# krisbrud/gym-auv

Hardware: AMD Instinct MI355X
Metric: env-steps/sec (higher is better)
Workload: dtype f64; 1 GPU; 4096 envs x 180 sensors per GPU, 50 static polygon obstacles (BASELINE configs[2]); envs_per_gpu=4096, n_sensors=180, total_envs=4096, parallelism=env-shard x1 (no step-path collective), ranks=1, hipgraph_steps=0, steps_per_launch=64, sub_batches=1, api=multi, step_mode=one_launch, roofline_step_mode=one_launch, actions=uniform, worlds_per_env=2, collective_backend=none, episodes_finished=212

## Files before the change

gym_auv_amd/csrc/k_step_fused.hip:

```cpp
#include <cstdlib>
#include <hip/hip_ext.h>

#define AUV_DEVICE_FUNCS_ONLY
#include "auv_multi_geom.h"
#include "k1_dynamics.hip"
#include "k2_lidar.hip"
#include "k3_nav_reward.hip"

#ifndef AUV_K23_MIN_WAVES
#define AUV_K23_MIN_WAVES 4
#endif

#ifdef AUV_TEST_HOOKS
#define AUV_HOOK_SKEW(d) ((d).pair_skew)
#define AUV_HOOK_FAULT(d) ((d).pair_fault)
#else
#define AUV_HOOK_SKEW(d) 0
#define AUV_HOOK_FAULT(d) 0
#endif

namespace {

#define PAIR_EMPTY AUV_PAIR_EMPTY
#define PAIR_COLLISION AUV_PAIR_COLLISION
// ... 13 lines not shown
  }
}

__device__ __forceinline__ void pair_publish_lidar(const AuvDev& d, const int e, const int lane, const int collision,
                                                   const double term) {
  auv_stores_done();
  if (AUV_HOOK_FAULT(d) == 1 && e == d.e0) return;
  if (lane == 0)
    __hip_atomic_store(d.pair_word + e, collision ? PAIR_COLLISION : (unsigned long long)__double_as_longlong(term),
                       __ATOMIC_RELAXED, __HIP_MEMORY_SCOPE_AGENT);
}

__global__ void __launch_bounds__(AUV_BLOCK, AUV_K23_MIN_WAVES) k23_lidar_nav(AuvDev dk, float* __restrict__ obs_out) {
  const AuvDev& d = dk;
  extern __shared__ __align__(16) unsigned char smem[];
  const int lane = threadIdx.x;
  const int ne = d.ne;
  if ((int)blockIdx.x >= ne) {
    const int el = (int)blockIdx.x - ne;
    if (el >= ne) return;
    const int e = auv_uniform(d.e0 + el);
#ifdef AUV_STAMPS
    const unsigned long long t_nav0 = wall_clock64();
#endif
    k3_nav_env(d, e, lane, smem, obs_out);
#ifdef AUV_STAMPS
    if (lane == 0) d.stamps[(size_t)e * 16 + 12] = t_nav0, d.stamps[(size_t)e * 16 + 13] = wall_clock64();
#endif
  } else {
    const int e = auv_uniform(d.e0 + (int)blockIdx.x);
    if (e == d.e0 && lane == 0 && dk.ring_slots > 1 && dk.ring_slot_host == -1) *dk.ring_pos = (*dk.ring_pos + 1) % dk.ring_slots;
    const Slice L = carve(smem, d);
    AUV_STAMP_DECL
#ifdef AUV_STAMPS
    const unsigned long long t_real0 = wall_clock64();
#endif
    int2 lim0 = make_int2(INT32_MIN, INT32_MIN);
    const int n_act = k2_front(d, e, lane, L, 1, nullptr, 0, nullptr, false, d.cfg.use_lidar ? &lim0 : nullptr);
    if (d.cfg.use_lidar) {
      AUV_STAMP()
#ifdef AUV_STAMPS
      unsigned long long sub[4] = {0, 0, 0, 0};
      k2_stage_and_pairs(d, L, lane, n_act, d.state[2 * (size_t)d.n + e], sub);
      if (lane == 0) d.stamps[(size_t)e * 16 + 7] = sub[0], d.stamps[(size_t)e * 16 + 14] = sub[1], d.stamps[(size_t)e * 16 + 15] = sub[2], d.stamps[(size_t)e * 16 + 6] = sub[3];
#else
      k2_stage_and_pairs(d, L, lane, n_act, d.state[2 * (size_t)d.n + e]);
#endif
      AUV_STAMP()
      double term = 0.0;
      k2_back(d, e, lane, L, n_act, obs_out, &term, &lim0);
      AUV_STAMP()
      AUV_STAMP_FLUSH(e, 0)
#ifdef AUV_STAMPS
      if (lane == 0) d.stamps[(size_t)e * 16 + 3] = t_real0, d.stamps[(size_t)e * 16 + 4] = wall_clock64();
      if (lane == 0) d.stamps[(size_t)e * 16 + 5] = (unsigned long long)L.sbase[n_act];
#endif
    }
  }
}

__device__ __forceinline__ double pair_lane_value(const unsigned long long v, const int src) {
  const unsigned lo = (unsigned)__builtin_amdgcn_readlane((int)(unsigned)v, src);
  const unsigned hi = (unsigned)__builtin_amdgcn_readlane((int)(unsigned)(v >> 32), src);
  return __longlong_as_double((long long)(((unsigned long long)hi << 32) | lo));
}

#define ROLES_MAGIC 0x9e3779b97f4a7c15ull
__device__ __forceinline__ unsigned long long roles_mark(const unsigned long long x) { return (x ^ ROLES_MAGIC) | 1ull; }

__device__ __forceinline__ unsigned long long roles_group_xor(const unsigned long long w) {
  int lo = (int)(unsigned)w, hi = (int)(unsigned)(w >> 32);
  lo ^= __builtin_amdgcn_update_dpp(0, lo, 0xB1, 0xF, 0xF, true), hi ^= __builtin_amdgcn_update_dpp(0, hi, 0xB1, 0xF, 0xF, true);
  lo ^= __builtin_amdgcn_update_dpp(0, lo, 0x4E, 0xF, 0xF, true), hi ^= __builtin_amdgcn_update_dpp(0, hi, 0x4E, 0xF, 0xF, true);
  lo ^= __builtin_amdgcn_update_dpp(0, lo, 0x141, 0xF, 0xF, true), hi ^= __builtin_amdgcn_update_dpp(0, hi, 0x141, 0xF, 0xF, true);
  return ((unsigned long long)(unsigned)hi << 32) | (unsigned)lo;
}

__device__ __forceinline__ unsigned long long roles_lane_word(const unsigned long long v, const int src) {
  return ((unsigned long long)(unsigned)__builtin_amdgcn_readlane((int)(unsigned)(v >> 32), src) << 32) |
         (unsigned)__builtin_amdgcn_readlane((int)(unsigned)v, src);
}

__device__ __forceinline__ unsigned long long roles_tagmix(const unsigned long long tag) { return tag * 0xd6e8feb86659fd93ull; }
__device__ __forceinline__ int roles_wait_state(const AuvDev& d, const int e, const int lane, EnvPre& pre, const unsigned long long tagmix = 0ull,
                                                const bool have_first = false, const unsigned long long v_first = 0ull) {
  const unsigned long long* pk = d.k1_pkt + 8 * (size_t)e;
  unsigned long long v = 0;
  for (int polls = 0;; polls++) {
    if (have_first && polls == 0) v = v_first;
    else v = __hip_atomic_load(pk + (lane & 7), __ATOMIC_RELAXED, __HIP_MEMORY_SCOPE_AGENT);
    const unsigned long long got = roles_lane_word(v, 7);
    if (got != 0ull) {
      unsigned long long x = roles_lane_word(v, 0);
#pragma unroll
      for (int i = 1; i < 7; i++) x ^= roles_lane_word(v, i);
      if (roles_mark(x ^ tagmix) == got) break;
    }
    if (polls == (AUV_HOOK_FAULT(d) ? (1 << 12) : PAIR_POLL_LIMIT)) {
      if (lane == 0) auv_st<true>(d.broken + e, (uint8_t)1);
      roles_give_up(d, d.e0, d.ne, 2, lane);
      return 1;
    }
    __builtin_amdgcn_s_sleep(ROLES_POLL_SLEEP);
  }
#pragma unroll
  for (int i = 0; i < 6; i++) pre.s[i] = pair_lane_value(v, i);
  pre.cnt.y = (int)__builtin_amdgcn_readlane((int)(unsigned)v, 6);
  return (unsigned)pre.cnt.y == ROLES_ABORT_COUNTER ? 2 : 0;
}

__device__ __forceinline__ void roles_publish_search(const AuvDev& d, const int e, const int lane, const NavNear& nr, const unsigned long long tagmix = 0ull) {
  unsigned long long* h = d.nav_hand + 8 * (size_t)e;
  const unsigned long long w0 = (unsigned long long)__double_as_longlong(nr.A.x), w1 = (unsigned long long)__double_as_longlong(nr.A.y),
                           w2 = (unsigned long long)__double_as_longlong(nr.B.x), w3 = (unsigned long long)__double_as_longlong(nr.B.y),
                           w4 = (unsigned long long)__double_as_longlong(nr.cum);
  if (AUV_HOOK_FAULT(d) == 3 && e == d.e0) return;
  if (lane == 0) {
    __hip_atomic_store(h + 0, w0, __ATOMIC_RELAXED, __HIP_MEMORY_SCOPE_AGENT), __hip_atomic_store(h + 1, w1, __ATOMIC_RELAXED, __HIP_MEMORY_SCOPE_AGENT);
    __hip_atomic_store(h + 2, w2, __ATOMIC_RELAXED, __HIP_MEMORY_SCOPE_AGENT), __hip_atomic_store(h + 3, w3, __ATOMIC_RELAXED, __HIP_MEMORY_SCOPE_AGENT);
    __hip_atomic_store(h + 4, w4, __ATOMIC_RELAXED, __HIP_MEMORY_SCOPE_AGENT);
    __hip_atomic_store(h + 7, roles_mark(w0 ^ w1 ^ w2 ^ w3 ^ w4 ^ tagmix), __ATOMIC_RELAXED, __HIP_MEMORY_SCOPE_AGENT);
  }
}

__device__ __forceinline__ unsigned long long roles_group_word(const unsigned long long v, const int src) {
  const unsigned lo = (unsigned)__shfl((int)(unsigned)v, src, K1_GROUP), hi = (unsigned)__shfl((int)(unsigned)(v >> 32), src, K1_GROUP);
  return ((unsigned long long)hi << 32) | lo;
}
__device__ __forceinline__ double roles_group_value(const unsigned long long v, const int src) {
  return __longlong_as_double((long long)roles_group_word(v, src));
}
__device__ __forceinline__ bool roles_record_ok(const unsigned long long v, const int c, const unsigned long long tagmix = 0ull) {
  const unsigned long long x = roles_group_xor(c < 7 ? v : 0ull), mark = roles_group_word(v, 7);
  return mark != 0ull && roles_mark(x ^ tagmix) == mark;
}

__device__ __forceinline__ void roles_finish_wave(const AuvDev& dk, const int f, const int lane, float* __restrict__ obs_out,
                                                  float* __restrict__ reward_out, uint8_t* __restrict__ done_out) {
  const __attribute__((address_space(4))) AuvDev* dc = (const __attribute__((address_space(4))) AuvDev*)dk.self;
  const AuvDev& d = *(const AuvDev*)dc;
  StepTabs st;
  st.cfg.min_cumulative_reward = dc->cfg.min_cumulative_reward, st.cfg.min_goal_distance = dc->cfg.min_goal_distance;
  st.cfg.min_path_progress = dc->cfg.min_path_progress, st.cfg.look_ahead_distance = dc->cfg.look_ahead_distance;
  st.cfg.max_timesteps = dc->cfg.max_timesteps, st.cfg.rewarder = dc->cfg.rewarder, st.cfg.test_mode = dc->cfg.test_mode;
  st.cfg.auto_reset = dc->cfg.auto_reset, st.cfg.n_sensors = dc->cfg.n_sensors, st.cfg.use_lidar = dc->cfg.use_lidar;
  st.cfg.obs_channels = dc->cfg.obs_channels, st.pool_ns = dc->pool_ns;
  st.knot_s = dc->knot_s, st.knot_coef = dc->knot_coef;
  st.info64 = dc->info64, st.nav64 = dc->nav64, st.obs64 = dc->obs64, st.rew_path = dc->rew_path, st.reward64 = dc->reward64;
  st.step_info = dc->step_info, st.episode = dc->episode, st.ep_log = dc->ep_log, st.ep_log_count = dc->ep_log_count;
  st.ep_log_cap = dc->ep_log_cap, st.world_idx = dc->world_idx, st.counters = dc->counters;
  st.fw_serial = dc->fw_serial, st.n = dc->n;
  st.ring_slots = 1, st.ring_slot_host = 0, st.ring_pos = nullptr;
  unsigned long long* const pair_word = dc->pair_word;
  unsigned long long* const k1_pkt = dc->k1_pkt;
  unsigned long long* const nav_hand = dc->nav_hand;
  const EnvDesc* const env_desc = dc->env_desc;
  const double* const world_scalar = dc->world_scalar;
  double* const state = dc->state;
  const int n_envs = dc->n;
  const int ne = dk.ne, e0 = dk.e0;
  const int g = lane / K1_GROUP, c = lane % K1_GROUP;
  const int er = 8 * (8 * (f / 8) + g) + (f % 8);
  const bool live = er < ne;
  const int e = e0 + (live ? er : ne - 1);
  int4 cnt = st.counters[e];
  const int w = st.world_idx[e];
  const double cum_in = st.info64[8 * (size_t)e + 4], cte_sum_in = st.info64[8 * (size_t)e + 7];
  const EnvDesc ed = env_desc[e];
  TailIn t;
  t.kn0 = ed.kn0, t.nk = ed.nk;
  {
    const double* ws = world_scalar + 8 * (size_t)ed.w;
    t.L = ws[0], t.goal_x = ws[1], t.goal_y = ws[2];
    t.knot_first = st.knot_s[ed.kn0], t.knot_last = st.knot_s[ed.kn0 + ed.nk - 1];
    t.maxp_in = st.info64[8 * (size_t)e + 5];
  }
  const unsigned long long* pk = k1_pkt + 8 * (size_t)e;
  unsigned long long* hd = nav_hand + 8 * (size_t)e;
  const int limit = AUV_HOOK_FAULT(dk) ? (1 << 12) : PAIR_POLL_LIMIT;
#ifdef AUV_STAMPS
// ... 128 lines not shown
    if (b - nk >= ne) return;
    const int e = auv_uniform(d.e0 + b - nk);
#ifdef AUV_STAMPS
    if (lane == 0) d.stamps[(size_t)e * 16 + 3] = wall_clock64();
#endif
    if (auv_uniform(*d.abort_flag)) return;
    ed = d.env_desc[e];
    pre.cnt = d.counters[e];
    pre.ed = &ed;
    const Slice L = carve(smem, d);
    k2_movers<true>(d, e, lane, L, ed, 1);
    const K2Pre kp = k2_prefetch(d, e, lane, ed);
    k2_stage_beams(d, lane, L);
#ifdef AUV_STAMPS
    if (lane == 0) d.stamps[(size_t)e * 16 + 1] = wall_clock64();
#endif
    {
      const int ws = roles_wait_state(d, e, lane, pre);
      if (ws) {
        if (ws == 2 && ed.M > 0 && lane == 0) auv_st<true>(d.broken + e, (uint8_t)1);
        return;
      }
    }
#ifdef AUV_STAMPS
    if (lane == 0) d.stamps[(size_t)e * 16 + 2] = wall_clock64();
#endif
    int n_act = 0;
    int2 lim0 = make_int2(INT32_MIN, INT32_MIN);
    if (AUV_RUN_L(d, 1)) n_act = k2_front<true>(d, e, lane, L, 1, &pre, 1, &kp, true, &lim0);
#ifdef AUV_STAMPS
    if (lane == 0) d.stamps[(size_t)e * 16 + 8] = wall_clock64();
#endif
    if (AUV_RUN_L(d, 3)) k2_stage_and_pairs(d, L, lane, n_act, pre.s[2]);
#ifdef AUV_STAMPS
    if (lane == 0) d.stamps[(size_t)e * 16 + 11] = wall_clock64();
#endif
    double term = 0.0;
    const int collision = k2_back<true>(d, e, lane, L, n_act, obs_out, &term, &lim0);
#ifdef AUV_STAMPS
    if (lane == 0) d.stamps[(size_t)e * 16 + 4] = wall_clock64();
#endif
    pair_publish_lidar(d, e, lane, collision, term);
#ifdef AUV_STAMPS
    if (lane == 0) d.stamps[(size_t)e * 16 + 14] = wall_clock64();
#endif
  } else if (b < nk + 2 * nb + AUV_HOOK_SKEW(d)) {
    const int el = b - nk - nb - AUV_HOOK_SKEW(d);
    if (el < 0 || el >= ne) return;
    const int e = auv_uniform(d.e0 + el);
    ed = d.env_desc[e];
    pre.cnt = d.counters[e];
    pre.ed = &ed;
#ifdef AUV_STAMPS
    if (lane == 0) d.stamps[(size_t)e * 16 + 12] = wall_clock64();
#endif
    if (roles_wait_state(d, e, lane, pre)) return;
#ifdef AUV_STAMPS
    if (lane == 0) d.stamps[(size_t)e * 16 + 5] = wall_clock64();
#endif
    NavNear nr;
    nr.A = nr.B = make_double2(0.0, 0.0), nr.cum = 0.0;
    if (AUV_RUN_N(d, 1)) {
      int* list = (int*)smem;
      const NavSpec sp = nav_bounds(d, e, lane, list, pre.s[0], pre.s[1], &ed);
      if (AUV_RUN_N(d, 2)) nr = nav_nearest(d, e, lane, list, pre.s[0], pre.s[1], sp);
    }
    roles_publish_search(d, e, lane, nr);
#ifdef AUV_STAMPS
    if (lane == 0) d.stamps[(size_t)e * 16 + 6] = wall_clock64();
#endif
  } else {
    const int f = b - nk - 2 * nb - AUV_HOOK_SKEW(d);
    if (f < 0 || f >= nk) return;
    __builtin_amdgcn_s_setprio(2);
    roles_finish_wave(d, f, lane, obs_out, reward_out, done_out);
  }
}

#define CARRY_WORDS 24

#ifdef AUV_STAMPS_MULTI
#define MSTAMP(e, k) do { if (lane == 0) stamp[(size_t)(e) * 16 + (k)] = wall_clock64(); } while (0)
#define MSTAMP_IF(cond, e, k) do { if (cond) stamp[(size_t)(e) * 16 + (k)] = wall_clock64(); } while (0)
#define MSTAMP_PARAM , unsigned long long* stamp
#define MSTAMP_ARG , stamp
#else
#define MSTAMP(e, k) do { } while (0)
#define MSTAMP_IF(cond, e, k) do { } while (0)
#define MSTAMP_PARAM
#define MSTAMP_ARG
#endif

__device__ __forceinline__ unsigned long long carry_ed_word(const EnvDesc& ed, const int i) {
  switch (i) {
    case 0: return (unsigned long long)ed.k0;
    case 1: return (unsigned long long)ed.m0;
    case 2: return (unsigned long long)ed.p0;
    case 3: return (unsigned long long)ed.c0;
    case 4: return (unsigned long long)ed.kn0;
    case 5: return (unsigned long long)(unsigned)ed.K | ((unsigned long long)(unsigned)ed.M << 32);
    case 6: return (unsigned long long)(unsigned)ed.P | ((unsigned long long)(unsigned)ed.nch << 32);
    default: return (unsigned long long)(unsigned)ed.nk | ((unsigned long long)(unsigned)ed.w << 32);
  }
}
__device__ __forceinline__ void carry_ed_from(EnvDesc& ed, const unsigned long long w[8]) {
  ed.k0 = (long long)w[0], ed.m0 = (long long)w[1], ed.p0 = (long long)w[2], ed.c0 = (long long)w[3], ed.kn0 = (long long)w[4];
  ed.K = (int)(unsigned)w[5], ed.M = (int)(unsigned)(w[5] >> 32), ed.P = (int)(unsigned)w[6], ed.nch = (int)(unsigned)(w[6] >> 32);
  ed.nk = (int)(unsigned)w[7], ed.w = (int)(unsigned)(w[7] >> 32);
}

__device__ __forceinline__ int carry_wait_wave(const AuvDev& d, const int e, const int lane, const unsigned long long tagmix, EnvDesc& ed, int4& cnt) {
  const unsigned long long* cw = d.carry + CARRY_WORDS * (size_t)e;
  unsigned long long v = 0ull;
  for (int polls = 0;; polls++) {
    if (lane < CARRY_WORDS) v = __hip_atomic_load(cw + lane, __ATOMIC_RELAXED, __HIP_MEMORY_SCOPE_AGENT);
    const unsigned long long ma = roles_lane_word(v, 7), mb = roles_lane_word(v, 20);
    if (ma != 0ull && mb != 0ull) {
      unsigned long long xa = roles_lane_word(v, 0), xb = roles_lane_word(v, 8);
#pragma unroll
      for (int i = 1; i < 7; i++) xa ^= roles_lane_word(v, i);
#pragma unroll
      for (int i = 9; i < 20; i++) xb ^= roles_lane_word(v, i);
      if (roles_mark(xa ^ tagmix) == ma && roles_mark(xb ^ tagmix) == mb) break;
    }
    if ((polls & 31) == 31 && auv_uniform(__hip_atomic_load(d.abort_flag, __ATOMIC_RELAXED, __HIP_MEMORY_SCOPE_AGENT))) return 2;
    if (polls == (AUV_HOOK_FAULT(d) ? (1 << 12) : PAIR_POLL_LIMIT)) {
      if (lane == 0) auv_st<true>(d.broken + e, (uint8_t)1);
      roles_give_up(d, d.e0, d.ne, 6, lane);
      return 1;
    }
    __builtin_amdgcn_s_sleep(ROLES_POLL_SLEEP);
  }
  unsigned long long w[8];
#pragma unroll
  for (int i = 0; i < 8; i++) w[i] = roles_lane_word(v, 12 + i);
  carry_ed_from(ed, w);
  const unsigned long long c6 = roles_lane_word(v, 6), c8 = roles_lane_word(v, 8);
  cnt = make_int4((int)(unsigned)c6, (int)(unsigned)(c6 >> 32), (int)(unsigned)c8, 0);
  return 0;
}

template <bool MULTI>
__device__ __forceinline__ void roles_finish_wave_multi(const AuvDev& dk, const int f, const int lane, float* __restrict__ obs_out,
                                                        float* __restrict__ reward_out, uint8_t* __restrict__ done_out, const int step,
                                                        const bool last_step, const unsigned long long tagmix, const unsigned long long tagmix_prev MSTAMP_PARAM) {
  const __attribute__((address_space(4))) AuvDev* dc = (const __attribute__((address_space(4))) AuvDev*)dk.self;
  const AuvDev& d = *(const AuvDev*)dc;
  StepTabs st;
  st.cfg.min_cumulative_reward = dc->cfg.min_cumulative_reward, st.cfg.min_goal_distance = dc->cfg.min_goal_distance;
  st.cfg.min_path_progress = dc->cfg.min_path_progress, st.cfg.look_ahead_distance = dc->cfg.look_ahead_distance;
  st.cfg.max_timesteps = dc->cfg.max_timesteps, st.cfg.rewarder = dc->cfg.rewarder, st.cfg.test_mode = dc->cfg.test_mode;
  st.cfg.auto_reset = dc->cfg.auto_reset, st.cfg.n_sensors = dc->cfg.n_sensors, st.cfg.use_lidar = dc->cfg.use_lidar;
  st.cfg.obs_channels = dc->cfg.obs_channels, st.pool_ns = dc->pool_ns;
  st.knot_s = dc->knot_s, st.knot_coef = dc->knot_coef;
  st.info64 = dc->info64, st.nav64 = dc->nav64, st.obs64 = dc->obs64, st.rew_path = dc->rew_path, st.reward64 = dc->reward64;
  st.step_info = dc->step_info, st.episode = dc->episode, st.ep_log = dc->ep_log, st.ep_log_count = dc->ep_log_count;
  st.ep_log_cap = dc->ep_log_cap, st.world_idx = dc->world_idx, st.counters = dc->counters;
  st.fw_serial = nullptr, st.n = dc->n;
  st.ring_slots = 1, st.ring_slot_host = 0, st.ring_pos = nullptr;
  unsigned long long* const pair_word = dc->pair_word;
  unsigned long long* const k1_pkt = dc->k1_pkt;
  unsigned long long* const nav_hand = dc->nav_hand;
  unsigned long long* const carry = dc->carry;
  const EnvDesc* const env_desc = dc->env_desc;
  const double* const world_scalar = dc->world_scalar;
  double* const state = dc->state;
  uint8_t* const broken = dc->broken;
  const int n_envs = dc->n;
  const int ne = dk.ne, e0 = dk.e0;
  const int g = lane / K1_GROUP, c = lane % K1_GROUP;
  const int er = 8 * (8 * (f / 8) + g) + (f % 8);
  const bool live = er < ne;
  const int e = e0 + (live ? er : ne - 1);
  const int limit = AUV_HOOK_FAULT(dk) ? (1 << 12) : PAIR_POLL_LIMIT;
  int4 cnt;
  double cum_in, cte_sum_in, maxp_in;
  EnvDesc ed;
  unsigned long long* const cw = carry + CARRY_WORDS * (size_t)e;
  if (step == 0) {
    cnt = st.counters[e];
    cum_in = st.info64[8 * (size_t)e + 4], cte_sum_in = st.info64[8 * (size_t)e + 7], maxp_in = st.info64[8 * (size_t)e + 5];
    ed = env_desc[e];
  } else {
    unsigned long long v0 = 0ull, v1 = 0ull, v2 = 0ull;
    bool ok = !live;
    for (int polls = 0;; polls++) {
      if (!ok) {
        v0 = __hip_atomic_load(cw + c, __ATOMIC_RELAXED, __HIP_MEMORY_SCOPE_AGENT);
        v1 = __hip_atomic_load(cw + 8 + c, __ATOMIC_RELAXED, __HIP_MEMORY_SCOPE_AGENT);
        v2 = __hip_atomic_load(cw + 16 + c, __ATOMIC_RELAXED, __HIP_MEMORY_SCOPE_AGENT);
      }
      const unsigned long long xb = roles_group_xor(v1) ^ roles_group_xor(c < 4 ? v2 : 0ull), mb = roles_group_word(v2, 4);
      ok = !live || (roles_record_ok(v0, c, tagmix_prev) && mb != 0ull && roles_mark(xb ^ tagmix_prev) == mb);
      if (!__any(!ok)) break;
      if ((polls & 31) == 31 && auv_uniform(__hip_atomic_load(dc->abort_flag, __ATOMIC_RELAXED, __HIP_MEMORY_SCOPE_AGENT))) return;
      if (polls == limit) {
        if (live && c == 0) auv_st<true>(broken + e, (uint8_t)1);
        roles_give_up(d, e0, ne, 6, lane);
        return;
      }
      __builtin_amdgcn_s_sleep(ROLES_POLL_SLEEP);
    }
    const unsigned long long c6 = roles_group_word(v0, 6), c8 = roles_group_word(v1, 0);
    cnt = make_int4((int)(unsigned)c6, (int)(unsigned)(c6 >> 32), (int)(unsigned)c8, 0);
    cum_in = roles_group_value(v1, 1), maxp_in = roles_group_value(v1, 2), cte_sum_in = roles_group_value(v1, 3);
    unsigned long long w[8];
#pragma unroll
    for (int i = 0; i < 4; i++) w[i] = roles_group_word(v1, 4 + i);
#pragma unroll
    for (int i = 0; i < 4; i++) w[4 + i] = roles_group_word(v2, i);
    carry_ed_from(ed, w);
    if (!live) ed = env_desc[e];
  }
  const int w = ed.w;
  TailIn t;
  t.kn0 = ed.kn0, t.nk = ed.nk;
  {
    const double* ws = world_scalar + 8 * (size_t)ed.w;
    t.L = ws[0], t.goal_x = ws[1], t.goal_y = ws[2];
    t.knot_first = st.knot_s[ed.kn0], t.knot_last = st.knot_s[ed.kn0 + ed.nk - 1];
    t.maxp_in = maxp_in;
  }
  const unsigned long long* pk = k1_pkt + 8 * (size_t)e;
  unsigned long long* hd = nav_hand + 8 * (size_t)e;
  unsigned long long vp = 0ull, vh = 0ull;
  bool okp = !live, okh = !live, aborted = false;
  for (int polls = 0;; polls++) {
    if (!okp) vp = __hip_atomic_load(pk + c, __ATOMIC_RELAXED, __HIP_MEMORY_SCOPE_AGENT);
    if (!okh) vh = __hip_atomic_load(hd + c, __ATOMIC_RELAXED, __HIP_MEMORY_SCOPE_AGENT);
    okp = !live || roles_record_ok(vp, c, tagmix);
    aborted = live && okp && (unsigned)roles_group_word(vp, 6) == ROLES_ABORT_COUNTER;
    okh = !live || aborted || roles_record_ok(vh, c, tagmix);
    if (!__any(!(okp && okh))) break;
    if (polls == limit) {
      if (live && c == 0) auv_st<true>(broken + e, (uint8_t)1);
      roles_give_up(d, e0, ne, 3, lane);
      return;
    }
    __builtin_amdgcn_s_sleep(ROLES_POLL_SLEEP);
  }
  if (__any(aborted)) return;
  t.px = roles_group_value(vp, 0), t.py = roles_group_value(vp, 1), t.psi = roles_group_value(vp, 2);
  t.u = roles_group_value(vp, 3), t.v = roles_group_value(vp, 4), t.r = roles_group_value(vp, 5);
  cnt.y = (int)(unsigned)roles_group_word(vp, 6);
  t.nr.A = make_double2(roles_group_value(vh, 0), roles_group_value(vh, 1));
  t.nr.B = make_double2(roles_group_value(vh, 2), roles_group_value(vh, 3));
  t.nr.cum = roles_group_value(vh, 4);
  NavOut no;
  no.rew_path = no.reached = no.goal = no.progress = no.u = no.v = no.r = no.cte100 = no.maxp = 0.0;
  unsigned long long word = live ? __hip_atomic_load(pair_word + e, __ATOMIC_RELAXED, __HIP_MEMORY_SCOPE_AGENT) : 0ull;
  no = nav_tail<K1_GROUP>(st, e, c, live, t, obs_out);
  if (live && c < 6) state[(size_t)c * (size_t)n_envs + e] = __longlong_as_double((long long)vp);
  for (int polls = 0;; polls++) {
    if (!__any(word == PAIR_EMPTY)) break;
    if (word == PAIR_EMPTY) word = __hip_atomic_load(pair_word + e, __ATOMIC_RELAXED, __HIP_MEMORY_SCOPE_AGENT);
    if (!__any(word == PAIR_EMPTY)) break;
    if (polls == limit) {
      if (live && c == 0) auv_st<true>(broken + e, (uint8_t)1);
      roles_give_up(d, e0, ne, 1, lane);
      return;
    }
    __builtin_amdgcn_s_sleep(ROLES_POLL_SLEEP);
  }
  MSTAMP_IF(live && c == 0, e, 14);
  int do_reset = 0;
  double co[2] = {0.0, 0.0};
  if (live && c == 0) {
    __hip_atomic_store(pair_word + e, PAIR_EMPTY, __ATOMIC_RELAXED, __HIP_MEMORY_SCOPE_AGENT);
    __hip_atomic_store(k1_pkt + 8 * (size_t)e + 7, 0ull, __ATOMIC_RELAXED, __HIP_MEMORY_SCOPE_AGENT);
    __hip_atomic_store(hd + 7, 0ull, __ATOMIC_RELAXED, __HIP_MEMORY_SCOPE_AGENT);
    RewardIn in;
    const int collision = word == PAIR_COLLISION;
    in.closeness_reward = collision ? 0.0 : __longlong_as_double((long long)word);
    in.path_reward = no.rew_path, in.reached = no.reached, in.goal = no.goal, in.progress = no.progress;
    in.u = no.u, in.v = no.v, in.yaw_rate = no.r;
    in.cum = cum_in;
    in.cte100 = no.cte100, in.cte_sum = cte_sum_in;
    st.info64[8 * (size_t)e] = collision;
    do_reset = reward_apply(st, e, collision, cnt, in, reward_out, done_out, false, co);
  }
  unsigned long long m = __ballot(do_reset);
  const unsigned long long m_reset = m;
  while (m) {
    const int src = __ffsll((long long)m) - 1;
    m &= m - 1;
    const int er2 = auv_uniform(__shfl(e, src, AUV_WAVE));
    const int wr = auv_uniform(__shfl(w, src, AUV_WAVE)), ep = auv_uniform(__shfl(cnt.z, src, AUV_WAVE));
    const AuvDev* dp = dk.self;
    asm volatile("" : "+s"(dp));
    const AuvDev& dr = *(const AuvDev*)(const __attribute__((address_space(4))) AuvDev*)dp;
    restore_env<false, true>(dr, er2, (int)(((long long)wr + dr.n) % dr.n_worlds), lane, ep, obs_out);
  }
  if (last_step) return;
  auv_stores_done();
  unsigned long long w0, w1, w2;
  {
    const int cx = __shfl(cnt.x, 0, K1_GROUP), cy = __shfl(cnt.y, 0, K1_GROUP), cz = __shfl(cnt.z, 0, K1_GROUP);
    const double cum = __shfl(co[0], 0, K1_GROUP), cte = __shfl(co[1], 0, K1_GROUP), maxp = __shfl(no.maxp, 0, K1_GROUP);
    w0 = c < 6 ? vp : (unsigned long long)(unsigned)cx | ((unsigned long long)(unsigned)cy << 32);
    w1 = c == 0 ? (unsigned long long)(unsigned)cz
                : (c == 1 ? (unsigned long long)__double_as_longlong(cum)
                          : (c == 2 ? (unsigned long long)__double_as_longlong(maxp) : (c == 3 ? (unsigned long long)__double_as_longlong(cte) : carry_ed_word(ed, c - 4))));
    w2 = c < 4 ? carry_ed_word(ed, 4 + c) : 0ull;
  }
  if (m_reset & (0xffull << (8 * g))) {
    const size_t n = (size_t)n_envs;
    const int4 rc = make_int4(0, 0, __shfl(cnt.z, 0, K1_GROUP), 0);
    const EnvDesc ne_ = auv_make_desc<true>(d, (int)(((long long)w + d.n) % d.n_worlds));
    const double sv = c < 6 ? __hip_atomic_load(state + (size_t)c * n + e, __ATOMIC_RELAXED, __HIP_MEMORY_SCOPE_AGENT) : 0.0;
    const double iv = (c >= 1 && c <= 3) ? __hip_atomic_load(st.info64 + 8 * (size_t)e + (c == 1 ? 4 : (c == 2 ? 5 : 7)), __ATOMIC_RELAXED, __HIP_MEMORY_SCOPE_AGENT) : 0.0;
    w0 = c < 6 ? (unsigned long long)__double_as_longlong(sv) : 0ull;
    w1 = c == 0 ? (unsigned long long)(unsigned)rc.z : (c <= 3 ? (unsigned long long)__double_as_longlong(iv) : carry_ed_word(ne_, c - 4));
    w2 = c < 4 ? carry_ed_word(ne_, 4 + c) : 0ull;
  }
  const unsigned long long ma = roles_mark(roles_group_xor(c < 7 ? w0 : 0ull) ^ tagmix);
  const unsigned long long mb = roles_mark(roles_group_xor(w1) ^ roles_group_xor(c < 4 ? w2 : 0ull) ^ tagmix);
  if (live) {
    __hip_atomic_store(cw + c, c < 7 ? w0 : ma, __ATOMIC_RELAXED, __HIP_MEMORY_SCOPE_AGENT);
    __hip_atomic_store(cw + 8 + c, w1, __ATOMIC_RELAXED, __HIP_MEMORY_SCOPE_AGENT);
    __hip_atomic_store(cw + 16 + c, c < 4 ? w2 : (c == 4 ? mb : 0ull), __ATOMIC_RELAXED, __HIP_MEMORY_SCOPE_AGENT);
  }
}

#define AUV_KERNARG_DESC(name)                                                                                                                       \
  const __attribute__((address_space(4))) void* name##_kp_ = (const __attribute__((address_space(4))) void*)__builtin_amdgcn_kernarg_segment_ptr(); \
  asm volatile("" : "+s"(name##_kp_));                                                                                                               \
  const AuvDev& name = *(const AuvDev*)(const __attribute__((address_space(4))) AuvDev*)name##_kp_

__global__ void __launch_bounds__(AUV_WAVE, AUV_K23_MIN_WAVES) k_step_multi(AuvDev dk, const void* __restrict__ actions, float* __restrict__ obs_out,
                                                                           float* __restrict__ reward_out, uint8_t* __restrict__ done_out,
                                                                           const int n_steps, const int first_slot, const int n_slots,
                                                                           const unsigned long long seq0, const int lead_dyn, const int lag_fin, const unsigned magic_c) {
  AUV_KERNARG_DESC(d);
#define STEP_MULTI_REC 0
#include "k_step_multi_body.inc"
#undef STEP_MULTI_REC
}

__global__ void __launch_bounds__(AUV_WAVE, AUV_K23_MIN_WAVES) k_step_record(AuvDev dk, const void* __restrict__ actions, float* __restrict__ obs_out,
                                                                            float* __restrict__ reward_out, uint8_t* __restrict__ done_out,
                                                                            const int n_steps, const int first_slot, const int n_slots,
                                                                            const unsigned long long seq0, const int lead_dyn, const int lag_fin, const unsigned magic_c,
                                                                            const unsigned long long obs_stride, const unsigned long long reward_stride,
                                                                            const unsigned long long done_stride) {
  AUV_KERNARG_DESC(d);
#define STEP_MULTI_REC 1
#include "k_step_multi_body.inc"
#undef STEP_MULTI_REC
}

__global__ void __launch_bounds__(256) k_record_last(const float* __restrict__ obs_last, const float* __restrict__ reward_last,
                                                     const uint8_t* __restrict__ done_last, float* __restrict__ obs, float* __restrict__ reward,
                                                     uint8_t* __restrict__ done, const int e0, const int ne, const int D, const int32_t* __restrict__ abort_flag) {
  if (*abort_flag) return;
  const size_t i = (size_t)blockIdx.x * 256 + threadIdx.x;
  const size_t o0 = (size_t)e0 * (size_t)D;
  if (obs_last && i < (size_t)ne * (size_t)D) obs[o0 + i] = obs_last[o0 + i];
  if (i < (size_t)ne) reward[e0 + i] = reward_last[e0 + i], done[e0 + i] = done_last[e0 + i];
}

__global__ void __launch_bounds__(AUV_WAVE) k31_reward_dyn(AuvDev d, const void* __restrict__ actions, float* __restrict__ obs_out,
                                                           float* __restrict__ reward_out, uint8_t* __restrict__ done_out) {
  const int lane = threadIdx.x;
  const int e = blockIdx.x * AUV_WAVE + lane;
  int do_reset = 0, w = 0;
  int4 cnt = make_int4(0, 0, 0, 0);
  if (e < d.n) {
    cnt = d.counters[e];
    w = d.world_idx[e];
    const int collision = d.collision[e];
    d.info64[8 * (size_t)e] = collision;
    do_reset = reward_block(d, e, collision, cnt, false, 0.0, nullptr, reward_out, done_out, false);
  }
  unsigned long long m = __ballot(do_reset);
  const bool any_reset = m != 0;
  while (m) {
    const int src = __ffsll((long long)m) - 1;
    m &= m - 1;
    const int er = auv_uniform(__shfl(e, src, AUV_WAVE));
    const int wr = auv_uniform(__shfl(w, src, AUV_WAVE)), ep = __shfl(cnt.z, src, AUV_WAVE);
    restore_env(d, er, auv_next_world_wave(d, wr, lane), lane, ep, obs_out);
  }
  if (any_reset) __builtin_amdgcn_fence(__ATOMIC_ACQ_REL, "workgroup");
  if (e < d.n) k1_env(d, e, actions, true);
}

__global__ void __launch_bounds__(AUV_WAVE) k_probe_order(unsigned int* __restrict__ words, int np, int nc, unsigned int tag,
                                                          unsigned int* __restrict__ failures) {
  extern __shared__ __align__(16) unsigned char smem[];
  const int b = (int)blockIdx.x, lane = threadIdx.x;
  if (lane == 0) smem[0] = 1;
  unsigned int* mine = words + b;
  const unsigned int* src = nullptr;
  if (b >= np + 2 * nc) {
    const int q = b - np - 2 * nc;
    if (lane < 8) src = words + np + nc + 8 * q + lane;
    else if (lane < 16) src = words + np + 8 * q + (lane - 8);
    else if (lane < 24) src = words + (8 * q + (lane - 16)) % np;
  } else if (b >= np + nc) src = words + np + (b - np - nc);
  else if (b >= np) src = words + (b - np) % np;
  if (b >= np) {
    int polls = 0;
    for (;;) {
      const bool there = !src || __hip_atomic_load(src, __ATOMIC_RELAXED, __HIP_MEMORY_SCOPE_AGENT) == tag;
// ... 146 lines not shown
```

gym_auv_amd/csrc/k_step_multi_body.inc:

```
  extern __shared__ __align__(16) unsigned char smem[];
#ifdef AUV_STAMPS_MULTI
  const unsigned long long t_entry = wall_clock64();
#endif
  const int lane = threadIdx.x;
  const int ne = d.ne;
  const bool cohorts = lead_dyn >= 0;
  const AuvMultiWave wa = auv_multi_decode_steps(blockIdx.x, ne, n_steps);
  const AuvMultiWave wc = auv_multi_decode_cohorts(blockIdx.x, ne, n_steps, lead_dyn, lag_fin, magic_c);
  const int step = auv_uniform(cohorts ? wc.step : wa.step);
  const int role = auv_uniform(cohorts ? wc.role : wa.role), bi = auv_uniform(cohorts ? wc.bi : wa.bi);
  if (step >= n_steps) return;
#if STEP_MULTI_REC
  {
    obs_out += (unsigned long long)(unsigned)step * obs_stride;
    reward_out += (unsigned long long)(unsigned)step * reward_stride;
    done_out += (unsigned long long)(unsigned)step * done_stride;
  }
#endif
  const unsigned long long tagmix = roles_tagmix(seq0 + (unsigned long long)step + 1ull), tagmix_prev = roles_tagmix(seq0 + (unsigned long long)step);
#ifdef AUV_STAMPS_MULTI
  unsigned long long* const stamp = d.stamps + (step == n_steps / 2 ? (size_t)0 : (size_t)16 * (size_t)d.n);
#endif
  if (role == 0) {
    __builtin_amdgcn_s_setprio(3);
    const int b = bi;
    const int g = lane / K1_GROUP, c = lane % K1_GROUP;
    const int er = 8 * (8 * (b / 8) + g) + (b % 8);
    const bool live = er < ne;
    const int eg = d.e0 + (live ? er : ne - 1);
    int y, gave_up = 0;
    double y0 = 0.0;
    MSTAMP_IF(live && c == 0, eg, 10);
    const int ab_early = __hip_atomic_load(d.abort_flag, __ATOMIC_RELAXED, __HIP_MEMORY_SCOPE_AGENT);
    double act0, act1;
    k1_action(d, actions, eg, &act0, &act1, (first_slot + step) % n_slots);
    if (step == 0) {
      y = d.counters[eg].y + 1;
    } else {
      const unsigned long long* cw = d.carry + CARRY_WORDS * (size_t)eg;
      unsigned long long v = 0ull;
      bool ok = !live;
      for (int polls = 0;; polls++) {
        if (!ok) v = __hip_atomic_load(cw + c, __ATOMIC_RELAXED, __HIP_MEMORY_SCOPE_AGENT);
        ok = !live || roles_record_ok(v, c, tagmix_prev);
        if (!__any(!ok)) break;
        if ((polls & 31) == 31 && auv_uniform(__hip_atomic_load(d.abort_flag, __ATOMIC_RELAXED, __HIP_MEMORY_SCOPE_AGENT))) {
          gave_up = 1;
          break;
        }
        if (polls == (AUV_HOOK_FAULT(d) ? (1 << 12) : PAIR_POLL_LIMIT)) {
          if (live && c == 0) auv_st<true>(d.broken + eg, (uint8_t)1);
          roles_give_up(d, d.e0, d.ne, 6, lane);
          gave_up = 1;
          break;
        }
        __builtin_amdgcn_s_sleep(ROLES_POLL_SLEEP);
      }
      y0 = __longlong_as_double((long long)v);
      y = (int)(unsigned)(roles_group_word(v, 6) >> 32) + 1;
    }
    const int aborted = gave_up | auv_uniform(ab_early);
    double t = 0.0;
    MSTAMP_IF(live && c == 0, eg, 11);
    const double2 act = make_double2(act0, act1);
    if (!aborted) t = k1_group(d, actions, eg, lane, step == 0 ? nullptr : &y0, (first_slot + step) % n_slots, &act);
    unsigned long long* pk = d.k1_pkt + 8 * (size_t)eg;
    const unsigned long long word = aborted ? (c == 6 ? (unsigned long long)ROLES_ABORT_COUNTER : 0ull)
                                            : (c < 6 ? (unsigned long long)__double_as_longlong(t) : (c == 6 ? (unsigned long long)(unsigned)y : 0ull));
    const unsigned long long mark = roles_mark(roles_group_xor(word) ^ tagmix);
    if (live && !(AUV_HOOK_FAULT(d) == 2 && eg == d.e0 && step == 0))
      __hip_atomic_store(pk + c, c < 7 ? word : mark, __ATOMIC_RELAXED, __HIP_MEMORY_SCOPE_AGENT);
    MSTAMP_IF(live && c == 0, eg, 12);
    return;
  }
  EnvPre pre;
  EnvDesc ed;
  if (role == 1) {
    const int e = auv_uniform(d.e0 + bi);
    MSTAMP(e, 0);
    const int ab_early = __hip_atomic_load(d.abort_flag, __ATOMIC_RELAXED, __HIP_MEMORY_SCOPE_AGENT);
    const unsigned long long pk_first = __hip_atomic_load(d.k1_pkt + 8 * (size_t)e + (lane & 7), __ATOMIC_RELAXED, __HIP_MEMORY_SCOPE_AGENT);
    const Slice L = carve(smem, d);
    K2Pre kp;
    if (step == 0) {
      ed = d.env_desc[e];
      pre.cnt = d.counters[e];
      pre.ed = &ed;
      if (auv_uniform(ab_early)) return;
      k2_movers<true>(d, e, lane, L, ed, 1);
      kp = k2_prefetch(d, e, lane, ed);
    } else {
      if (carry_wait_wave(d, e, lane, tagmix_prev, ed, pre.cnt)) return;
      if (auv_uniform(ab_early)) return;
      pre.ed = &ed;
      k2_movers<true, true>(d, e, lane, L, ed, 1);
      kp = k2_prefetch<true>(d, e, lane, ed);
    }
    k2_stage_beams(d, lane, L);
    {
      const int ws = roles_wait_state(d, e, lane, pre, tagmix, true, pk_first);
      if (ws) {
        if (ws == 2 && ed.M > 0 && lane == 0) auv_st<true>(d.broken + e, (uint8_t)1);
        return;
      }
    }
    MSTAMP(e, 2);
    int2 lim0 = make_int2(INT32_MIN, INT32_MIN);
    const int n_act = k2_front<true>(d, e, lane, L, 1, &pre, 1, &kp, true, &lim0);
    k2_stage_and_pairs(d, L, lane, n_act, pre.s[2]);
    MSTAMP(e, 4);
    double term = 0.0;
    const int collision = k2_back<true>(d, e, lane, L, n_act, obs_out, &term, &lim0);
    pair_publish_lidar(d, e, lane, collision, term);
    MSTAMP(e, 5);
#ifdef AUV_STAMPS_MULTI
    if (lane == 0) stamp[(size_t)e * 16 + 1] = t_entry;
    __builtin_amdgcn_s_waitcnt(0x0F70);
    MSTAMP(e, 3);
#endif
  } else if (role == 2) {
    const int e = auv_uniform(d.e0 + bi);
    MSTAMP(e, 6);
    const unsigned long long pk_first = __hip_atomic_load(d.k1_pkt + 8 * (size_t)e + (lane & 7), __ATOMIC_RELAXED, __HIP_MEMORY_SCOPE_AGENT);
    if (step == 0) {
      ed = d.env_desc[e];
      pre.cnt = d.counters[e];
    } else if (carry_wait_wave(d, e, lane, tagmix_prev, ed, pre.cnt)) {
      return;
    }
#ifdef AUV_STAMPS_MULTI
    if (lane == 0) stamp[(size_t)e * 16 + 7] = t_entry;
#endif
    pre.ed = &ed;
    if (roles_wait_state(d, e, lane, pre, tagmix, true, pk_first)) return;
    MSTAMP(e, 8);
    NavNear nr;
    int* list = (int*)smem;
    const NavSpec sp = nav_bounds(d, e, lane, list, pre.s[0], pre.s[1], &ed);
    nr = nav_nearest(d, e, lane, list, pre.s[0], pre.s[1], sp);
    roles_publish_search(d, e, lane, nr, tagmix);
    MSTAMP(e, 9);
  } else {
    const int f = bi;
    __builtin_amdgcn_s_setprio(2);
#ifdef AUV_STAMPS_MULTI
    const int fer = 8 * (8 * (f / 8) + lane / K1_GROUP) + (f % 8);
    const bool fst = fer < ne && lane % K1_GROUP == 0;
#endif
    MSTAMP_IF(fst, d.e0 + fer, 13);
    roles_finish_wave_multi<true>(d, f, lane, obs_out, reward_out, done_out, step, step == n_steps - 1, tagmix, tagmix_prev MSTAMP_ARG);
    MSTAMP_IF(fst, d.e0 + fer, 15);
  }
```

Measured before the change: 185.1 million env-steps/s.

## Fuse next-step dynamics into finish wave, drop dedicated dynamics waves after step 0

The finish wave now computes the next step's action and dynamics (k1_group) right after writing the carry, and publishes the k1 packet for the next step itself. Dynamics waves for steps after the first return immediately, which removes one cross-wave handoff (carry poll then k1 compute) from the per-step critical path. To keep waiting consumers from hanging when the finish wave exits early, abort propagation is added: abort_next writes an abort packet, and roles_wait_state gains a periodic abort-flag check. The cost is more work and register pressure in the finish wave, plus extra abort handling logic.

```diff
diff --git a/gym_auv_amd/csrc/k_step_fused.hip b/gym_auv_amd/csrc/k_step_fused.hip
--- a/gym_auv_amd/csrc/k_step_fused.hip
+++ b/gym_auv_amd/csrc/k_step_fused.hip
@@ -119,6 +119,7 @@
 }
 
 __device__ __forceinline__ unsigned long long roles_tagmix(const unsigned long long tag) { return tag * 0xd6e8feb86659fd93ull; }
+template <bool FLAG = false>
 __device__ __forceinline__ int roles_wait_state(const AuvDev& d, const int e, const int lane, EnvPre& pre, const unsigned long long tagmix = 0ull,
                                                 const bool have_first = false, const unsigned long long v_first = 0ull) {
   const unsigned long long* pk = d.k1_pkt + 8 * (size_t)e;
@@ -133,6 +134,7 @@
       for (int i = 1; i < 7; i++) x ^= roles_lane_word(v, i);
       if (roles_mark(x ^ tagmix) == got) break;
     }
+    if (FLAG && (polls & 31) == 31 && auv_uniform(__hip_atomic_load(d.abort_flag, __ATOMIC_RELAXED, __HIP_MEMORY_SCOPE_AGENT))) return 2;
     if (polls == (AUV_HOOK_FAULT(d) ? (1 << 12) : PAIR_POLL_LIMIT)) {
       if (lane == 0) auv_st<true>(d.broken + e, (uint8_t)1);
       roles_give_up(d, d.e0, d.ne, 2, lane);
@@ -427,8 +429,8 @@
 #ifdef AUV_STAMPS_MULTI
 #define MSTAMP(e, k) do { if (lane == 0) stamp[(size_t)(e) * 16 + (k)] = wall_clock64(); } while (0)
 #define MSTAMP_IF(cond, e, k) do { if (cond) stamp[(size_t)(e) * 16 + (k)] = wall_clock64(); } while (0)
-#define MSTAMP_PARAM , unsigned long long* stamp
-#define MSTAMP_ARG , stamp
+#define MSTAMP_PARAM , unsigned long long* stamp, unsigned long long* stamp_next
+#define MSTAMP_ARG , stamp, stamp_next
 #else
 #define MSTAMP(e, k) do { } while (0)
 #define MSTAMP_IF(cond, e, k) do { } while (0)
@@ -486,9 +488,10 @@
 }
 
 template <bool MULTI>
-__device__ __forceinline__ void roles_finish_wave_multi(const AuvDev& dk, const int f, const int lane, float* __restrict__ obs_out,
-                                                        float* __restrict__ reward_out, uint8_t* __restrict__ done_out, const int step,
-                                                        const bool last_step, const unsigned long long tagmix, const unsigned long long tagmix_prev MSTAMP_PARAM) {
+__device__ __forceinline__ void roles_finish_wave_multi(const AuvDev& dk, const int f, const int lane, const void* __restrict__ actions,
+                                                        float* __restrict__ obs_out, float* __restrict__ reward_out, uint8_t* __restrict__ done_out,
+                                                        const int step, const bool last_step, const int next_slot, const unsigned long long tagmix,
+                                                        const unsigned long long tagmix_prev, const unsigned long long tagmix_next MSTAMP_PARAM) {
   const __attribute__((address_space(4))) AuvDev* dc = (const __attribute__((address_space(4))) AuvDev*)dk.self;
   const AuvDev& d = *(const AuvDev*)dc;
   StepTabs st;
@@ -518,6 +521,11 @@
   const bool live = er < ne;
   const int e = e0 + (live ? er : ne - 1);
   const int limit = AUV_HOOK_FAULT(dk) ? (1 << 12) : PAIR_POLL_LIMIT;
+  auto abort_next = [&]() {
+    if (!last_step && live)
+      __hip_atomic_store(k1_pkt + 8 * (size_t)e + c, c < 6 ? 0ull : (c == 6 ? (unsigned long long)ROLES_ABORT_COUNTER : roles_mark((unsigned long long)ROLES_ABORT_COUNTER ^ tagmix_next)),
+                         __ATOMIC_RELAXED, __HIP_MEMORY_SCOPE_AGENT);
+  };
   int4 cnt;
   double cum_in, cte_sum_in, maxp_in;
   EnvDesc ed;
@@ -538,10 +546,14 @@
       const unsigned long long xb = roles_group_xor(v1) ^ roles_group_xor(c < 4 ? v2 : 0ull), mb = roles_group_word(v2, 4);
       ok = !live || (roles_record_ok(v0, c, tagmix_prev) && mb != 0ull && roles_mark(xb ^ tagmix_prev) == mb);
       if (!__any(!ok)) break;
-      if ((polls & 31) == 31 && auv_uniform(__hip_atomic_load(dc->abort_flag, __ATOMIC_RELAXED, __HIP_MEMORY_SCOPE_AGENT))) return;
+      if ((polls & 31) == 31 && auv_uniform(__hip_atomic_load(dc->abort_flag, __ATOMIC_RELAXED, __HIP_MEMORY_SCOPE_AGENT))) {
+        abort_next();
+        return;
+      }
       if (polls == limit) {
         if (live && c == 0) auv_st<true>(broken + e, (uint8_t)1);
         roles_give_up(d, e0, ne, 6, lane);
+        abort_next();
         return;
       }
       __builtin_amdgcn_s_sleep(ROLES_POLL_SLEEP);
@@ -558,6 +570,7 @@
     if (!live) ed = env_desc[e];
   }
   const int w = ed.w;
+  const unsigned long long ed_w1 = last_step ? 0ull : carry_ed_word(ed, c < 4 ? 0 : c - 4), ed_w2 = last_step ? 0ull : carry_ed_word(ed, c < 4 ? 4 + c : 7);
   TailIn t;
   t.kn0 = ed.kn0, t.nk = ed.nk;
   {
@@ -577,14 +590,22 @@
     aborted = live && okp && (unsigned)roles_group_word(vp, 6) == ROLES_ABORT_COUNTER;
     okh = !live || aborted || roles_record_ok(vh, c, tagmix);
     if (!__any(!(okp && okh))) break;
+    if ((polls & 1023) == 1023 && auv_uniform(__hip_atomic_load(dc->abort_flag, __ATOMIC_RELAXED, __HIP_MEMORY_SCOPE_AGENT))) {
+      abort_next();
+      return;
+    }
     if (polls == limit) {
       if (live && c == 0) auv_st<true>(broken + e, (uint8_t)1);
       roles_give_up(d, e0, ne, 3, lane);
+      abort_next();
       return;
     }
     __builtin_amdgcn_s_sleep(ROLES_POLL_SLEEP);
   }
-  if (__any(aborted)) return;
+  if (__any(aborted)) {
+    abort_next();
+    return;
+  }
   t.px = roles_group_value(vp, 0), t.py = roles_group_value(vp, 1), t.psi = roles_group_value(vp, 2);
   t.u = roles_group_value(vp, 3), t.v = roles_group_value(vp, 4), t.r = roles_group_value(vp, 5);
   cnt.y = (int)(unsigned)roles_group_word(vp, 6);
@@ -600,9 +621,15 @@
     if (!__any(word == PAIR_EMPTY)) break;
     if (word == PAIR_EMPTY) word = __hip_atomic_load(pair_word + e, __ATOMIC_RELAXED, __HIP_MEMORY_SCOPE_AGENT);
     if (!__any(word == PAIR_EMPTY)) break;
+    if ((polls & 1023) == 1023 && auv_uniform(__hip_atomic_load(dc->abort_flag, __ATOMIC_RELAXED, __HIP_MEMORY_SCOPE_AGENT))) {
+      if (live && c == 0) auv_st<true>(broken + e, (uint8_t)1);
+      abort_next();
+      return;
+    }
     if (polls == limit) {
       if (live && c == 0) auv_st<true>(broken + e, (uint8_t)1);
       roles_give_up(d, e0, ne, 1, lane);
+      abort_next();
       return;
     }
     __builtin_amdgcn_s_sleep(ROLES_POLL_SLEEP);
@@ -637,6 +664,13 @@
     restore_env<false, true>(dr, er2, (int)(((long long)wr + dr.n) % dr.n_worlds), lane, ep, obs_out);
   }
   if (last_step) return;
+#ifdef AUV_STAMPS_MULTI
+  MSTAMP_IF(live && c == 0, e, 15);
+  if (live && c == 0) stamp_next[(size_t)e * 16 + 10] = wall_clock64();
+#endif
+  const int ab_next = __hip_atomic_load(dc->abort_flag, __ATOMIC_RELAXED, __HIP_MEMORY_SCOPE_AGENT);
+  double act0, act1;
+  k1_action(d, actions, e, &act0, &act1, next_slot);
   auv_stores_done();
   unsigned long long w0, w1, w2;
   {
@@ -645,8 +679,8 @@
     w0 = c < 6 ? vp : (unsigned long long)(unsigned)cx | ((unsigned long long)(unsigned)cy << 32);
     w1 = c == 0 ? (unsigned long long)(unsigned)cz
                 : (c == 1 ? (unsigned long long)__double_as_longlong(cum)
-                          : (c == 2 ? (unsigned long long)__double_as_longlong(maxp) : (c == 3 ? (unsigned long long)__double_as_longlong(cte) : carry_ed_word(ed, c - 4))));
-    w2 = c < 4 ? carry_ed_word(ed, 4 + c) : 0ull;
+                          : (c == 2 ? (unsigned long long)__double_as_longlong(maxp) : (c == 3 ? (unsigned long long)__double_as_longlong(cte) : ed_w1)));
+    w2 = c < 4 ? ed_w2 : 0ull;
   }
   if (m_reset & (0xffull << (8 * g))) {
     const size_t n = (size_t)n_envs;
@@ -665,6 +699,24 @@
     __hip_atomic_store(cw + 8 + c, w1, __ATOMIC_RELAXED, __HIP_MEMORY_SCOPE_AGENT);
     __hip_atomic_store(cw + 16 + c, c < 4 ? w2 : (c == 4 ? mb : 0ull), __ATOMIC_RELAXED, __HIP_MEMORY_SCOPE_AGENT);
   }
+  __builtin_amdgcn_s_setprio(3);
+  if (auv_uniform(ab_next)) {
+    abort_next();
+    return;
+  }
+  const int y_next = (int)(unsigned)(roles_group_word(w0, 6) >> 32) + 1;
+  const double y0 = __longlong_as_double((long long)w0);
+  const double2 act = make_double2(act0, act1);
+#ifdef AUV_STAMPS_MULTI
+  if (live && c == 0) stamp_next[(size_t)e * 16 + 11] = wall_clock64();
+#endif
+  const double tn = k1_group(d, actions, e, lane, &y0, next_slot, &act);
+  const unsigned long long pw = c < 6 ? (unsigned long long)__double_as_longlong(tn) : (c == 6 ? (unsigned long long)(unsigned)y_next : 0ull);
+  const unsigned long long pm = roles_mark(roles_group_xor(pw) ^ tagmix_next);
+  if (live) __hip_atomic_store(k1_pkt + 8 * (size_t)e + c, c < 7 ? pw : pm, __ATOMIC_RELAXED, __HIP_MEMORY_SCOPE_AGENT);
+#ifdef AUV_STAMPS_MULTI
+  if (live && c == 0) stamp_next[(size_t)e * 16 + 12] = wall_clock64();
+#endif
 }
 
 #define AUV_KERNARG_DESC(name)                                                                                                                       \
diff --git a/gym_auv_amd/csrc/k_step_multi_body.inc b/gym_auv_amd/csrc/k_step_multi_body.inc
--- a/gym_auv_amd/csrc/k_step_multi_body.inc
+++ b/gym_auv_amd/csrc/k_step_multi_body.inc
@@ -10,6 +10,7 @@
   const int step = auv_uniform(cohorts ? wc.step : wa.step);
   const int role = auv_uniform(cohorts ? wc.role : wa.role), bi = auv_uniform(cohorts ? wc.bi : wa.bi);
   if (step >= n_steps) return;
+  if (role == 0 && step > 0) return;
 #if STEP_MULTI_REC
   {
     obs_out += (unsigned long long)(unsigned)step * obs_stride;
@@ -20,6 +21,7 @@
   const unsigned long long tagmix = roles_tagmix(seq0 + (unsigned long long)step + 1ull), tagmix_prev = roles_tagmix(seq0 + (unsigned long long)step);
 #ifdef AUV_STAMPS_MULTI
   unsigned long long* const stamp = d.stamps + (step == n_steps / 2 ? (size_t)0 : (size_t)16 * (size_t)d.n);
+  unsigned long long* const stamp_next = d.stamps + (step + 1 == n_steps / 2 ? (size_t)0 : (size_t)16 * (size_t)d.n);
 #endif
   if (role == 0) {
     __builtin_amdgcn_s_setprio(3);
@@ -28,47 +30,21 @@
     const int er = 8 * (8 * (b / 8) + g) + (b % 8);
     const bool live = er < ne;
     const int eg = d.e0 + (live ? er : ne - 1);
-    int y, gave_up = 0;
-    double y0 = 0.0;
     MSTAMP_IF(live && c == 0, eg, 10);
     const int ab_early = __hip_atomic_load(d.abort_flag, __ATOMIC_RELAXED, __HIP_MEMORY_SCOPE_AGENT);
     double act0, act1;
-    k1_action(d, actions, eg, &act0, &act1, (first_slot + step) % n_slots);
-    if (step == 0) {
-      y = d.counters[eg].y + 1;
-    } else {
-      const unsigned long long* cw = d.carry + CARRY_WORDS * (size_t)eg;
-      unsigned long long v = 0ull;
-      bool ok = !live;
-      for (int polls = 0;; polls++) {
-        if (!ok) v = __hip_atomic_load(cw + c, __ATOMIC_RELAXED, __HIP_MEMORY_SCOPE_AGENT);
-        ok = !live || roles_record_ok(v, c, tagmix_prev);
-        if (!__any(!ok)) break;
-        if ((polls & 31) == 31 && auv_uniform(__hip_atomic_load(d.abort_flag, __ATOMIC_RELAXED, __HIP_MEMORY_SCOPE_AGENT))) {
-          gave_up = 1;
-          break;
-        }
-        if (polls == (AUV_HOOK_FAULT(d) ? (1 << 12) : PAIR_POLL_LIMIT)) {
-          if (live && c == 0) auv_st<true>(d.broken + eg, (uint8_t)1);
-          roles_give_up(d, d.e0, d.ne, 6, lane);
-          gave_up = 1;
-          break;
-        }
-        __builtin_amdgcn_s_sleep(ROLES_POLL_SLEEP);
-      }
-      y0 = __longlong_as_double((long long)v);
-      y = (int)(unsigned)(roles_group_word(v, 6) >> 32) + 1;
-    }
-    const int aborted = gave_up | auv_uniform(ab_early);
+    k1_action(d, actions, eg, &act0, &act1, first_slot % n_slots);
+    const int y = d.counters[eg].y + 1;
+    const int aborted = auv_uniform(ab_early);
     double t = 0.0;
     MSTAMP_IF(live && c == 0, eg, 11);
     const double2 act = make_double2(act0, act1);
-    if (!aborted) t = k1_group(d, actions, eg, lane, step == 0 ? nullptr : &y0, (first_slot + step) % n_slots, &act);
+    if (!aborted) t = k1_group(d, actions, eg, lane, nullptr, first_slot % n_slots, &act);
     unsigned long long* pk = d.k1_pkt + 8 * (size_t)eg;
     const unsigned long long word = aborted ? (c == 6 ? (unsigned long long)ROLES_ABORT_COUNTER : 0ull)
                                             : (c < 6 ? (unsigned long long)__double_as_longlong(t) : (c == 6 ? (unsigned long long)(unsigned)y : 0ull));
     const unsigned long long mark = roles_mark(roles_group_xor(word) ^ tagmix);
-    if (live && !(AUV_HOOK_FAULT(d) == 2 && eg == d.e0 && step == 0))
+    if (live && !(AUV_HOOK_FAULT(d) == 2 && eg == d.e0))
       __hip_atomic_store(pk + c, c < 7 ? word : mark, __ATOMIC_RELAXED, __HIP_MEMORY_SCOPE_AGENT);
     MSTAMP_IF(live && c == 0, eg, 12);
     return;
@@ -98,7 +74,7 @@
     }
     k2_stage_beams(d, lane, L);
     {
-      const int ws = roles_wait_state(d, e, lane, pre, tagmix, true, pk_first);
+      const int ws = roles_wait_state<true>(d, e, lane, pre, tagmix, true, pk_first);
       if (ws) {
         if (ws == 2 && ed.M > 0 && lane == 0) auv_st<true>(d.broken + e, (uint8_t)1);
         return;
@@ -132,7 +108,7 @@
     if (lane == 0) stamp[(size_t)e * 16 + 7] = t_entry;
 #endif
     pre.ed = &ed;
-    if (roles_wait_state(d, e, lane, pre, tagmix, true, pk_first)) return;
+    if (roles_wait_state<true>(d, e, lane, pre, tagmix, true, pk_first)) return;
     MSTAMP(e, 8);
     NavNear nr;
     int* list = (int*)smem;
@@ -148,6 +124,7 @@
     const bool fst = fer < ne && lane % K1_GROUP == 0;
 #endif
     MSTAMP_IF(fst, d.e0 + fer, 13);
-    roles_finish_wave_multi<true>(d, f, lane, obs_out, reward_out, done_out, step, step == n_steps - 1, tagmix, tagmix_prev MSTAMP_ARG);
-    MSTAMP_IF(fst, d.e0 + fer, 15);
+    roles_finish_wave_multi<true>(d, f, lane, actions, obs_out, reward_out, done_out, step, step == n_steps - 1, (first_slot + step + 1) % n_slots,
+                                  tagmix, tagmix_prev, roles_tagmix(seq0 + (unsigned long long)step + 2ull) MSTAMP_ARG);
+    MSTAMP_IF(fst && step == n_steps - 1, d.e0 + fer, 15);
   }
```

New measurement: 182.3 million env-steps/s. -1.5%, worse.
